# BayesWatch/deep-kernel-transfer

Hardware: AMD Instinct MI355X
Metric: episodes/sec (higher is better)
Workload: dtype f32/f16x2-split

## Files before the change

### deep-kernel-transfer_amd/_lib.py

```python
from __future__ import annotations

import ctypes
import json
import os
import subprocess
import threading
from typing import NamedTuple, Optional

_HERE = os.path.dirname(os.path.abspath(__file__))
_ROOT = os.path.dirname(_HERE)
CSRC = os.path.join(_HERE, "csrc")
INCLUDE = os.path.join(_ROOT, "include")
SOURCES = ["dkt_gram.hip", "dkt_gram_ep.hip", "dkt_gram_big.hip", "dkt_gram_small.hip", "dkt_classkernel.hip", "dkt_mll.hip", "dkt_mll_mfma.hip", "dkt_mll_h2.hip", "dkt_mll_reg.hip", "dkt_mll_big.hip", "dkt_mll_tiled.hip", "dkt_mll_band.hip", "dkt_objective.hip", "dkt_predict.hip",
           "dkt_spectral.hip", "dkt_frontend.hip", "dkt_frontend_big.hip", "dkt_lowrank.hip", "dkt_mll_rownoise.hip", "dkt_laplace_grad.hip"]
OBJ_DIR = os.path.join(_HERE, "build")

_c_p = ctypes.c_void_p
_c_i = ctypes.c_int
_c_f = ctypes.c_float

SIGNATURES = {
    "dkt_abi_version": (_c_i, []),
    "dkt_device_cu_count": (_c_i, []),
    "dkt_reload_env": (None, []),
    "dkt_env_value": (ctypes.c_char_p, [ctypes.c_char_p]),
    "dkt_gram_f32": (_c_i, [_c_p, _c_p, _c_p, _c_i, _c_i, _c_i, _c_i, _c_i, _c_p, _c_p]),
    "dkt_mll_workspace_bytes": (ctypes.c_size_t, [_c_i, _c_i, _c_i]),
    "dkt_mll_workspace_bytes_for": (ctypes.c_size_t, [_c_i, _c_i, _c_i, ctypes.c_uint]),
    "dkt_mll_f32": (_c_i, [_c_p, _c_p, ctypes.c_long, _c_p, _c_p, _c_p, _c_i, _c_i, _c_i, _c_f, _c_i,
                           ctypes.c_uint, _c_p, _c_p, _c_p, _c_p, _c_p, _c_p, _c_p, _c_p, _c_p, _c_p,
                           _c_p, ctypes.c_size_t, _c_p]),
    "dkt_objective_f32": (_c_i, [_c_p, _c_p, _c_p, _c_i, _c_i, _c_p]),
    "dkt_hyper_grads_f32": (_c_i, [_c_p] * 8 + [_c_i, _c_i, _c_p]),
    "dkt_bn_param_grads_workspace_bytes": (ctypes.c_size_t, [_c_i, _c_i]),
    "dkt_bn_param_grads_f32": (_c_i, [_c_p, _c_p, _c_p, _c_p, _c_i, _c_i, _c_p, ctypes.c_size_t, _c_p]),
    "dkt_gram_bwd_f32": (_c_i, [_c_p, _c_p, _c_p, _c_i, _c_i, _c_i, _c_p, ctypes.c_uint, _c_p]),
    "dkt_rbf_bwd_f32": (_c_i, [_c_p, _c_p, _c_p, _c_p, _c_p, _c_i, _c_i, _c_p]),
    "dkt_sqdist_bwd_f32": (_c_i, [_c_p, _c_p, _c_p, _c_p, _c_p, _c_i, _c_i, _c_p]),
    "dkt_predict_f32": (_c_i, [_c_p, _c_p, _c_p, _c_p, _c_p, _c_p, _c_i, _c_i, _c_i, _c_i, _c_p]),
    "dkt_predict_per_class_f32": (_c_i, [_c_p, _c_p, _c_p, _c_p, _c_p, _c_p, _c_i, _c_i, _c_i, _c_i, _c_p]),
    "dkt_predict_var_f32": (_c_i, [_c_p, _c_p, _c_p, _c_p, _c_p, _c_p, _c_i, _c_i, _c_i, _c_i, _c_p]),
    "dkt_bn_stats_f32": (_c_i, [_c_p, _c_p, _c_p, _c_f, _c_p, _c_p, _c_p, _c_p, _c_p, _c_i, _c_i, _c_i, _c_p]),
    "dkt_gram_bn_f32": (_c_i, [_c_p, _c_p, _c_p, ctypes.c_long, _c_p, _c_p, _c_i, _c_i, _c_i, _c_p]),
    "dkt_gram_bn_train_f32": (_c_i, [_c_p, _c_p, _c_p, _c_f, _c_p, _c_p, _c_p, _c_p, _c_p, _c_p, _c_p, _c_i, _c_i, _c_i, _c_p]),
    "dkt_gram_bn_bwd_f32": (_c_i, [_c_p, _c_p, _c_p, _c_p, _c_p, ctypes.c_long, _c_p, _c_p, _c_p, _c_p, _c_p, _c_p, _c_p,
                                   _c_i, _c_i, _c_i, _c_p]),
    "dkt_affine_normalize_f32": (_c_i, [_c_p, _c_p, _c_p, ctypes.c_long, _c_p, _c_p, _c_i, _c_i, _c_i, _c_p]),
    "dkt_normalize_bn_bwd_f32": (_c_i, [_c_p, _c_p, _c_p, _c_p, ctypes.c_long, _c_p, _c_p, _c_p, _c_p, _c_p, _c_p, _c_p, _c_i, _c_i, _c_i, _c_p]),
    "dkt_class_kernel_f32": (_c_i, [_c_p, _c_i, _c_p, _c_i, _c_p, _c_i, _c_i, _c_i, _c_p]),
    "dkt_class_kernel_bwd_nsplit": (_c_i, [_c_i, _c_i]),
    "dkt_class_kernel_bwd_f32": (_c_i, [_c_p, _c_p, _c_i, _c_p, _c_i, _c_p, _c_p, _c_i, _c_i, _c_i, _c_p]),
# ... 550 lines not shown
```

### deep-kernel-transfer_amd/csrc/dkt_common.h

```cpp
#pragma once
#include <hip/hip_runtime.h>
#include <stdint.h>

typedef float f32x4 __attribute__((ext_vector_type(4)));
typedef float f32x16 __attribute__((ext_vector_type(16)));

#define DKT_WAVE 64

#include "dkt_env.h"
#include "dkt_lds_dense.h"

__device__ __forceinline__ float wave_sum(float v) {
#pragma unroll
    for (int o = 32; o > 0; o >>= 1) v += __shfl_down(v, o, DKT_WAVE);
    return v;
}

__device__ __forceinline__ float wave_allsum(float v) {
#pragma unroll
    for (int o = 32; o > 0; o >>= 1) v += __shfl_xor(v, o, DKT_WAVE);
    return v;
}

__device__ __forceinline__ float block_sum_256(float v, float* red) {
    v = wave_sum(v);
    __syncthreads();
    if ((threadIdx.x & 63) == 0) red[threadIdx.x >> 6] = v;
    __syncthreads();
    return red[0] + red[1] + red[2] + red[3];
}

__device__ __forceinline__ float4 load4_guard(const float* row, int col, int ncols, bool row_ok, bool vec_ok) {
    float4 v = make_float4(0.f, 0.f, 0.f, 0.f);
    if (!row_ok) return v;
    if (vec_ok) {
        if (col < ncols) v = *reinterpret_cast<const float4*>(row + col);
    } else {
        if (col + 0 < ncols) v.x = row[col + 0];
        if (col + 1 < ncols) v.y = row[col + 1];
        if (col + 2 < ncols) v.z = row[col + 2];
        if (col + 3 < ncols) v.w = row[col + 3];
    }
    return v;
}

static inline unsigned dkt_lds_pad(DktSwitch pad) { return (unsigned)dkt_env_int(pad, 0); }
```

### deep-kernel-transfer_amd/csrc/dkt_mll.h

```cpp
#pragma once
#include "dkt_common.h"
#include "../../include/dkt_abi.h"

struct MllArgs {
    const float* E;
    const float* Y;
    long y_bstride;
    const float* sv;
    const float* mean;
    const float* noise;
    const float* cls_weight;
    float* logp;
    float* alpha;
    float* L;
    float* W;
    float* dsv;
    float* dmean;
    float* dnoise;
    float* jitter_used;
    int32_t* info;
    float* ws;
    const int32_t* only_failed;
    int b0;
    int B, C, N, LD;
    float jitter0;
    int max_tries;
    unsigned flags;
    int p2_guard;
    float kappa_max = 0.f;
};

constexpr float DKT_HALF_LOG_2PI = 0.91893853320467274178f;
static_assert(DKT_HALF_LOG_2PI == dkt_lds::kHalfLog2Pi, "the two spellings of 1/2 log 2 pi round to one float");

bool dkt_mll_h2_serves(int N, unsigned flags);
void dkt_mll_h2_launch(const MllArgs& a, hipStream_t st);
bool dkt_mll_mfma_serves(int N, unsigned flags);
void dkt_mll_mfma_launch(const MllArgs& a, hipStream_t st);
bool dkt_mll_reg_launch(const MllArgs& a, hipStream_t st);

void dkt_chol_inv_block_launch(const float* A, int lda, long sA, float* L, int ldl, long sL, float* U, int ldu, long sU, int nb,
                               int pivot_base, int32_t* info, int nmat, hipStream_t st);
size_t dkt_mll_big_workspace_bytes(int B, int C, int N);
int dkt_mll_big_launch(const MllArgs& a, void* workspace, size_t ws_bytes, hipStream_t st);
bool dkt_mll_tiled_supports(int N, unsigned flags, int C = 1);
size_t dkt_mll_tiled_workspace_bytes(int B, int C, int N);
size_t dkt_mll_tiled_workspace_bytes_form(int B, int C, int N, bool per_class);
int dkt_mll_tiled_launch(const MllArgs& a, void* workspace, size_t ws_bytes, hipStream_t st);
bool dkt_mll_band_supports(int N, unsigned flags, int C);
bool dkt_mll_band_applies(int B, int C, int N, unsigned flags);
size_t dkt_mll_band_workspace_bytes(int B, int C, int N);
int dkt_mll_band_launch(const MllArgs& a, void* workspace, size_t ws_bytes, hipStream_t st);
void dkt_mll_generic_global_launch(MllArgs a, int b0, int count, float* ws, hipStream_t st);
size_t dkt_mll_generic_global_floats(int count, int N);
```

### deep-kernel-transfer_amd/csrc/dkt_mll.hip

```cpp
#include "dkt_mll.h"
#include <cstdint>
#include <cstdlib>

namespace {

constexpr size_t MLL_LDS_LIMIT = 150 * 1024;

__host__ __device__ inline int mll_ld(int N) { return N | 1; }
inline size_t mll_vec_floats(int N) { return (size_t)3 * (N + 1) + 32; }
inline size_t mll_mat_floats(int N) { return (size_t)(N + 1) * mll_ld(N); }
inline bool mll_fits_lds(int N) { return (mll_vec_floats(N) + mll_mat_floats(N)) * 4 <= MLL_LDS_LIMIT; }

template <bool GLOBAL>
__global__ __launch_bounds__(256) void mll_generic_kernel(MllArgs a) {
    extern __shared__ __attribute__((aligned(16))) float smem[];
    const int tid = threadIdx.x;
    const int tx = tid & 15, ty = tid >> 4;
    const int N = a.N, C = a.C, LD = a.LD, R = N + 1;
    const bool epc = (a.flags & DKT_MLL_E_PER_CLASS) != 0;
    const size_t unit = epc ? (size_t)a.b0 * C + blockIdx.x : (size_t)a.b0 + blockIdx.x;
    const int b = epc ? (int)(unit / (size_t)C) : (int)unit;
    const int c_first = epc ? (int)(unit % (size_t)C) : 0, c_end = epc ? c_first + 1 : C;
    if (a.only_failed) {
        bool need = false;
        for (int c = c_first; c < c_end; ++c) need = need || a.only_failed[(size_t)b * C + c] != 0;
        if (!need) return;
        __syncthreads();
    }
    float* cs = smem;
    float* ldiag = cs + R;
    float* al = ldiag + R;
    float* red = al + R;
    float* Mw = GLOBAL ? (a.ws + (size_t)blockIdx.x * R * LD) : (red + 32);
#define MW(p, j) Mw[(p) * LD + (j)]

    const float* Eb = a.E + unit * N * N;
    const bool want_grad = (a.flags & DKT_MLL_WANT_GRAD) != 0;
    const bool want_chol = (a.flags & DKT_MLL_WANT_CHOL) != 0;
    float* Wb = want_grad ? a.W + unit * N * N : nullptr;

    for (int c = c_first; c < c_end; ++c) {
        const float svc = a.sv[c], mc = a.mean[c], nzc = a.noise[c];
        const float* yc = a.Y + (size_t)b * a.y_bstride + (size_t)c * N;
        int fail_at = 0;
        float jit = 0.f;
        for (int attempt = 0; attempt <= a.max_tries; ++attempt) {
            jit = dkt_jitter_rung(a.jitter0, attempt);
            __syncthreads();
            for (int idx = tid; idx < N * N; idx += 256) {
                const int p = idx / N, j = idx - p * N;
                float v = 0.f;
                if (p >= j) {
// ... 91 lines not shown
                    const float mcv = 0.5f * (al[i] * al[j] - kinv);
                    const float e = Eb[(size_t)i * N + j];
                    if (i == j) { dsv_part += mcv * e; tr_part += mcv; }
                    else dsv_part += 2.0f * mcv * e;
                    const float wv = coef * mcv;
                    if (c == c_first) {
                        Wb[(size_t)i * N + j] = wv;
                        if (i != j) Wb[(size_t)j * N + i] = wv;
                    } else {
                        Wb[(size_t)i * N + j] += wv;
                        if (i != j) Wb[(size_t)j * N + i] += wv;
                    }
                }
            }
            const float dsv = block_sum_256(dsv_part, red);
            const float trm = block_sum_256(tr_part, red);
            if (tid == 0) {
                a.dsv[bc] = dsv;
                a.dmean[bc] = asum;
                a.dnoise[bc] = trm;
            }
        }
    }
#undef MW
}

}

size_t dkt_mll_generic_global_floats(int count, int N) { return (size_t)count * mll_mat_floats(N); }

void dkt_mll_generic_global_launch(MllArgs a, int b0, int count, float* ws, hipStream_t st) {
    a.b0 = b0; a.ws = ws; a.LD = mll_ld(a.N);
    const int units = (a.flags & DKT_MLL_E_PER_CLASS) ? count * a.C : count;
    hipLaunchKernelGGL(mll_generic_kernel<true>, dim3(units), dim3(256), mll_vec_floats(a.N) * sizeof(float), st, a);
}

constexpr float MLL_H2_KAPPA_MAX = 5.0e3f;

static int mll_status() { return hipGetLastError() == hipSuccess ? DKT_OK : DKT_ERR_LAUNCH; }
static int mll_generic_lds_launch(const MllArgs& a, hipStream_t st) {
    const size_t units = (size_t)a.B * ((a.flags & DKT_MLL_E_PER_CLASS) ? a.C : 1);
    const size_t lds = (mll_vec_floats(a.N) + mll_mat_floats(a.N)) * sizeof(float);
    if (lds > 48 * 1024 && hipFuncSetAttribute((const void*)mll_generic_kernel<false>, hipFuncAttributeMaxDynamicSharedMemorySize, (int)lds) != hipSuccess) return DKT_ERR_LAUNCH;
    hipLaunchKernelGGL(mll_generic_kernel<false>, dim3((unsigned)units), dim3(256), lds, st, a);
    return mll_status();
}

static int mll_p2_guard() { return dkt_env_int(DKT_SW_MLL_P2_GUARD, 1); }
static bool mll_force_f32mfma() { return dkt_env_is(DKT_SW_MLL_F32MFMA, '1'); }

enum class MllRoute { BadArg, H2, Mfma, Band, Tiled, Big, GenericLds, GenericGlobal };
struct MllPlan { MllRoute route; size_t ws_bytes; bool kappa_fixup; };

static MllPlan mll_plan(int B, int C, int N, unsigned flags, size_t avail_bytes) {
    if (B <= 0 || C <= 0 || N <= 0) return {MllRoute::BadArg, 0, false};
    const bool pc = (flags & DKT_MLL_E_PER_CLASS) != 0;
    const bool bad = (flags & DKT_MLL_FORCE_REG) || (pc && (flags & (DKT_MLL_WANT_CHOL | DKT_MLL_FORCE_F32MFMA | DKT_MLL_FORCE_BLOCKED)));
    if (mll_force_f32mfma() && !(flags & (DKT_MLL_E_PER_CLASS | DKT_MLL_FORCE_GENERIC | DKT_MLL_FORCE_REG | DKT_MLL_FORCE_BLOCKED))) flags |= DKT_MLL_FORCE_F32MFMA;
    const size_t gen = mll_fits_lds(N) ? 0 : (size_t)(pc ? (B < 128 ? B : 128) * C : B) * mll_mat_floats(N) * sizeof(float);
    MllPlan p = {mll_fits_lds(N) ? MllRoute::GenericLds : MllRoute::GenericGlobal, gen, false};
    size_t ws = 0;
    if (!(flags & DKT_MLL_FORCE_GENERIC)) {
        if (dkt_mll_h2_serves(N, flags)) p = {MllRoute::H2, 0, !(flags & DKT_MLL_NO_KAPPA_GUARD) && mll_fits_lds(N)};
        else if (dkt_mll_mfma_serves(N, flags)) p = {MllRoute::Mfma, 0, false};
        else if (dkt_mll_band_applies(B, C, N, flags) && (ws = dkt_mll_band_workspace_bytes(B, C, N)) <= avail_bytes) p = {MllRoute::Band, ws, false};
        else if (!(flags & DKT_MLL_FORCE_BLOCKED) && dkt_mll_tiled_supports(N, flags, C) && ((ws = dkt_mll_tiled_workspace_bytes_form(B, C, N, pc)) <= avail_bytes || pc))
            p = {MllRoute::Tiled, ws, false};
        else if (!pc && N + 1 > 128 && (ws = dkt_mll_big_workspace_bytes(B, C, N)) <= avail_bytes)
            p = {MllRoute::Big, ws > gen ? ws : gen, false};
    }
    if (bad) p.route = MllRoute::BadArg;
    return p;
}

extern "C" size_t dkt_mll_workspace_bytes(int B, int C, int N) {
    if (B <= 0 || N <= 0 || C <= 0) return 0;
    if (N + 1 <= 128) return 0;
    const size_t big = dkt_mll_big_workspace_bytes(B, C, N);
    const size_t gen = mll_fits_lds(N) ? 0 : (size_t)B * mll_mat_floats(N) * sizeof(float);
    const size_t til = dkt_mll_tiled_supports(N, 0) ? dkt_mll_tiled_workspace_bytes(B, C, N) : 0;
    const size_t bnd = dkt_mll_band_supports(N, 0, C) ? dkt_mll_band_workspace_bytes(B, C, N) : 0;
    size_t mx = big > gen ? big : gen;
    mx = mx > bnd ? mx : bnd;
    return mx > til ? mx : til;
}

extern "C" size_t dkt_mll_workspace_bytes_for(int B, int C, int N, unsigned flags) { return mll_plan(B, C, N, flags, SIZE_MAX).ws_bytes; }

extern "C" int dkt_mll_f32(const float* E, const float* Y, long y_bstride, const float* sv, const float* mean,
                           const float* noise, int B, int C, int N, float jitter0, int max_tries,
                           unsigned flags, const float* cls_weight, float* logp, float* alpha, float* L,
                           float* W, float* dsv, float* dmean, float* dnoise, float* jitter_used,
                           int32_t* info, void* workspace, size_t workspace_bytes, void* stream) {
    if (!E || !Y || !sv || !mean || !noise || !logp || !alpha || !jitter_used || !info) return DKT_ERR_BAD_ARG;
    if (B <= 0 || C <= 0 || N <= 0 || max_tries < 0 || max_tries > 8 || y_bstride < 0) return DKT_ERR_BAD_ARG;
    if ((flags & DKT_MLL_WANT_GRAD) && (!W || !dsv || !dmean || !dnoise)) return DKT_ERR_BAD_ARG;
    if ((flags & DKT_MLL_WANT_CHOL) && !L) return DKT_ERR_BAD_ARG;
    MllArgs a;
    a.E = E; a.Y = Y; a.y_bstride = y_bstride; a.sv = sv; a.mean = mean; a.noise = noise;
    a.cls_weight = cls_weight; a.logp = logp; a.alpha = alpha; a.L = L; a.W = W; a.dsv = dsv;
    a.dmean = dmean; a.dnoise = dnoise; a.jitter_used = jitter_used; a.info = info;
    a.ws = (float*)workspace; a.only_failed = nullptr; a.b0 = 0; a.B = B; a.C = C; a.N = N; a.LD = mll_ld(N);
    a.jitter0 = jitter0; a.max_tries = max_tries; a.flags = flags;
    a.p2_guard = mll_p2_guard();
    hipStream_t st = (hipStream_t)stream;
    const size_t avail = workspace ? workspace_bytes : 0;
    const MllPlan p = mll_plan(B, C, N, flags, avail);
    switch (p.route) {
        case MllRoute::BadArg: return DKT_ERR_BAD_ARG;
        case MllRoute::H2:
            a.kappa_max = p.kappa_fixup ? MLL_H2_KAPPA_MAX : 0.f;
            dkt_mll_h2_launch(a, st);
            if (!p.kappa_fixup) return mll_status();
            a.only_failed = a.info;
            return mll_generic_lds_launch(a, st);
        case MllRoute::Mfma: dkt_mll_mfma_launch(a, st); return mll_status();
        case MllRoute::Band: return dkt_mll_band_launch(a, workspace, workspace_bytes, st);
        case MllRoute::Tiled:
            if (avail < p.ws_bytes) return DKT_ERR_WORKSPACE;
            return dkt_mll_tiled_launch(a, workspace, workspace_bytes, st);
        case MllRoute::Big: return dkt_mll_big_launch(a, workspace, workspace_bytes, st);
        case MllRoute::GenericLds: return mll_generic_lds_launch(a, st);
        case MllRoute::GenericGlobal: {
            const size_t per_ep = (size_t)((flags & DKT_MLL_E_PER_CLASS) ? C : 1) * mll_mat_floats(N) * sizeof(float);
            const size_t fit = avail / per_ep;
            if (fit < 1) return DKT_ERR_WORKSPACE;
            const int cnt = fit < (size_t)B ? (int)fit : B;
            for (int b0 = 0; b0 < B; b0 += cnt) dkt_mll_generic_global_launch(a, b0, (B - b0 < cnt) ? B - b0 : cnt, (float*)workspace, st);
            return mll_status();
        }
    }
    return DKT_ERR_BAD_ARG;
}
```

### deep-kernel-transfer_amd/csrc/dkt_mll_h2.hip

```cpp
#include "dkt_wave_mll.h"
#include <cstdlib>

namespace {

using namespace dkt_mfma;

#ifndef DKT_H2E_P2H
#define DKT_H2E_P2H 1
#endif
#ifndef DKT_H2_SWEEP_PRIO
#define DKT_H2_SWEEP_PRIO 1
#endif

__device__ __forceinline__ void sweep_begin30(const f32x4 S, float (&x)[16], float& dv) {
#pragma unroll
    for (int q = 0; q < 4; ++q) spread_rows(S[q] * TWOM30, x[q], x[4 + q], x[8 + q], x[12 + q]);
    dv = 1.0f;
}

struct P1H2 : P1Base {
    h4 negIh;
};

struct ArithH2 {
// ... 409 lines not shown
            if (round + 1 < nrounds) __syncthreads();
        }
    }
    DKT_CLK(7);
#ifdef DKT_MFMA_CLOCKS
    DKT_CLK(8);
    if ((tid & 63) == 0 && a.ws) {
        unsigned long long* o = reinterpret_cast<unsigned long long*>(a.ws) + ((size_t)blockIdx.x * (MAX_WPG * EPW) + wall) * 48;
        for (int i = 0; i < 32; ++i) o[i] = clk[i];
        for (int i = 0; i < 16; ++i) o[32 + i] = clk2[i];
    }
#endif
}

template <int NT> constexpr int h2e_wlds() { return ntt(NT) < 19 ? ntt(NT) : 19; }

template <int NT>
__global__ __attribute__((amdgpu_flat_work_group_size(64, 64), amdgpu_waves_per_eu(2, 2)))
void mll_h2e_kernel(MllArgs a) {
    constexpr int WLDS = h2e_wlds<NT>();
    constexpr int WREG = ntt(NT) - WLDS;
    __shared__ f32x4 wl[WLDS * 64];
    __shared__ f32x4 yst[NT * 4];

    const bool epc = (a.flags & DKT_MLL_E_PER_CLASS) != 0;
    const bool want_grad = (a.flags & DKT_MLL_WANT_GRAD) != 0;
    const int C = a.C;
    const int b = epc ? (int)(blockIdx.x / (unsigned)C) : (int)blockIdx.x;
    const int c_first = epc ? (int)(blockIdx.x % (unsigned)C) : 0, c_end = epc ? c_first + 1 : C;
    const size_t mat = epc ? (size_t)b * C + c_first : (size_t)b;
    const float qnan = __int_as_float(0x7fc00000);
    int tq = threadIdx.x;
    DKT_OPAQUE_V(tq);
    int c16 = tq & 15, g4 = (tq >> 2) & 12, lane = tq & 63, N = a.N;
    DKT_OPAQUE_S(N);

    f32x4 wr[WREG > 0 ? WREG : 1];
#pragma unroll
    for (int n = 0; n < WREG; ++n) wr[n] = (f32x4){0.f, 0.f, 0.f, 0.f};
#pragma unroll
    for (int n = 0; n < WLDS; ++n) wl[n * 64 + lane] = (f32x4){0.f, 0.f, 0.f, 0.f};
#ifdef DKT_MFMA_CLOCKS
    unsigned long long ph[8] = {}, tprev = __builtin_amdgcn_s_memtime();
#define DKT_PH(i) do { __builtin_amdgcn_sched_barrier(0); const unsigned long long tn = __builtin_amdgcn_s_memtime(); ph[i] += tn - tprev; tprev = tn; __builtin_amdgcn_sched_barrier(0); } while (0)
#else
#define DKT_PH(i) do { } while (0)
// ... 387 lines not shown
        if (want_grad && !live && fail_at == 0) {
            float fro = 0.f;
#pragma unroll
            for (int j = 0; j < NT; ++j) {
#pragma unroll
                for (int i = 0; i <= j; ++i) {
#if DKT_H2E_P2H
                    const f32x4 u = join_h2(T.t[i][j]);
#else
                    const f32x4 u = T.t[i][j];
#endif
#pragma unroll
                    for (int q = 0; q < 4; ++q) fro += (j < NT - 1 || g4 + q < pN) ? u[q] * u[q] : 0.f;
                }
            }
#if DKT_H2E_P2H
            trk = wave_reduce_dpp<false>(fro) * ldexpf(1.0f, -2 * msc) / (gsc * gsc * unit2 * unit2) - aa;
#else
            trk = wave_reduce_dpp<false>(fro) * ldexpf(1.0f, -2 * msc) - aa;
#endif
        }
        if (lane == 0) {
            const bool ok = fail_at == 0;
            a.logp[bc] = ok ? (-0.5f * quad - 0.34657359027997264f * lsum - (float)N * DKT_HALF_LOG_2PI) : qnan;
            a.jitter_used[bc] = jit;
            a.info[bc] = (ok && kappa_high) ? -1 : fail_at;
            if (want_grad) {
                const float nz_eff = nzc + jit;
                a.dmean[bc] = ok ? asum : qnan;
                a.dnoise[bc] = ok ? -0.5f * trk : qnan;
                a.dsv[bc] = ok ? 0.5f * ((quad - (float)N) + nz_eff * trk) / svc : qnan;
            }
        }
        DKT_PH(5);
        attempt = 0;
        ++c;
    }
    if (want_grad) {
        tq = threadIdx.x;
        DKT_OPAQUE_V(tq);
        c16 = tq & 15; g4 = (tq >> 2) & 12; lane = tq & 63; N = a.N;
        DKT_OPAQUE_S(N);
        const int pN = N - 16 * (NT - 1);
        const float fin = poison ? qnan : ((sigma == 0.f) ? 0.f : sigma * ldexpf(1.0f, -2 * (15 - e_acc)));
        const brsrc Wr = mk_rsrc(a.W + mat * N * N, (unsigned)(N * N * 4));
#pragma unroll
        for (int j = 0; j < NT; ++j) {
            const bool col_ok = (j < NT - 1) || (c16 < pN);
#pragma unroll
            for (int i = 0; i <= j; ++i) {
                const int n = tidx(i, j);
                f32x4 v;
                if (n < WLDS) v = wl[n * 64 + lane];
                else v = wr[n - WLDS < 0 ? 0 : n - WLDS];
#pragma unroll
                for (int q = 0; q < 4; ++q) v[q] = poison ? qnan : v[q] * fin;
                if (i < j) {
                    bstore4(Wr, v, col_ok ? ((16 * j + c16) * N + 16 * i + g4) * 4 : OOB, 0);
#pragma unroll
                    for (int q = 0; q < 4; ++q) {
// ... 12 lines not shown
            }
        }
    }
#ifdef DKT_MFMA_CLOCKS
    DKT_PH(6);
    if (lane == 0 && a.ws) {
        unsigned long long* o = reinterpret_cast<unsigned long long*>(a.ws) + (size_t)blockIdx.x * 8;
        for (int i = 0; i < 7; ++i) o[i] = ph[i];
        o[7] = __builtin_amdgcn_s_getreg((4 << 0) | (0 << 6) | (31 << 11));
    }
#endif
}

int h2e_min_batch() { return dkt_env_int(DKT_SW_MLL_H2E_MINB, 1024); }

template <int NT>
void launch_h2(const MllArgs& a, hipStream_t st) {
    const bool g = (a.flags & DKT_MLL_WANT_GRAD) != 0;
    if constexpr (NT <= 7) {
        if (a.flags & DKT_MLL_E_PER_CLASS) {
            hipLaunchKernelGGL((mll_h2e_kernel<NT>), dim3(a.B * a.C), dim3(64), 0, st, a);
            return;
        }
        if (g && a.B >= h2e_min_batch()) {
            hipLaunchKernelGGL((mll_h2e_kernel<NT>), dim3(a.B), dim3(64), 0, st, a);
            return;
        }
    }
    const bool epc = (a.flags & DKT_MLL_E_PER_CLASS) != 0;
    const int rounds = (a.C + MAX_WPG - 1) / MAX_WPG;
    const int wpg = epc ? 1 : (a.C + rounds - 1) / rounds;
    constexpr int EPW = epw<NT>();
    const dim3 grid(((epc ? a.B * a.C : a.B) + EPW - 1) / EPW), block(64 * wpg * EPW);
    if (g && wpg == 5) hipLaunchKernelGGL((mll_h2_kernel<NT, true, true>), grid, block, 0, st, a, wpg);
    else if (g) hipLaunchKernelGGL((mll_h2_kernel<NT, true, false>), grid, block, 0, st, a, wpg);
    else hipLaunchKernelGGL((mll_h2_kernel<NT, false, false>), grid, block, 0, st, a, wpg);
}

}

bool dkt_mll_h2_serves(int N, unsigned flags) { return N + 1 <= 128 && !(flags & (DKT_MLL_WANT_CHOL | DKT_MLL_FORCE_F32MFMA)); }

void dkt_mll_h2_launch(const MllArgs& a, hipStream_t st) {
    switch ((a.N + 1 + 15) / 16) {
        case 1: launch_h2<1>(a, st); break;
        case 2: launch_h2<2>(a, st); break;
        case 3: launch_h2<3>(a, st); break;
        case 4: launch_h2<4>(a, st); break;
        case 5: launch_h2<5>(a, st); break;
        case 6: launch_h2<6>(a, st); break;
        case 7: launch_h2<7>(a, st); break;
        case 8: launch_h2<8>(a, st); break;
        default: break;
    }
}
```

### deep-kernel-transfer_amd/csrc/dkt_objective.hip

```cpp
#include "dkt_common.h"
#include "../../include/dkt_abi.h"

namespace {

__global__ __launch_bounds__(256) void objective_kernel(const float* __restrict__ logp, const float* __restrict__ cw, float* __restrict__ obj, const int B, const int C) {
    const int b = blockIdx.x * 256 + threadIdx.x;
    if (b >= B) return;
    float s = 0.f;
    for (int c = 0; c < C; ++c) s += (cw ? cw[c] : 1.0f) * logp[(size_t)b * C + c];
    obj[b] = s;
}

__global__ __launch_bounds__(256) void hyper_grads_kernel(const float* __restrict__ gobj, const float* __restrict__ cw, const float* __restrict__ d0, const float* __restrict__ d1,
                                                          const float* __restrict__ d2, float* __restrict__ g0, float* __restrict__ g1, float* __restrict__ g2, const int B,
                                                          const int C) {
    __shared__ float red[256];
    const int c = blockIdx.x, which = blockIdx.y, tid = threadIdx.x;
    const float* d = which == 0 ? d0 : (which == 1 ? d1 : d2);
    float* g = which == 0 ? g0 : (which == 1 ? g1 : g2);
    if (!d || !g) return;
    float s = 0.f;
    for (int b = tid; b < B; b += 256) s += gobj[b] * d[(size_t)b * C + c];
    red[tid] = s;
    __syncthreads();
#pragma unroll
    for (int w = 128; w > 0; w >>= 1) {
        if (tid < w) red[tid] += red[tid + w];
        __syncthreads();
    }
    if (tid == 0) g[c] = (cw ? cw[c] : 1.0f) * red[0];
}

// ... 85 lines not shown
```

### deep-kernel-transfer_amd/ops.py

```python
from __future__ import annotations

import ctypes
import os
import re
from typing import Optional

import torch

from . import _lib

KERNEL_LINEAR = 0
KERNEL_RBF = 1
KERNEL_SQDIST = 2
KERNEL_LINEAR_UNIT = 3
GRAM_UNIT_ROWS = 1
GRAM_W_SYMMETRIC = 2
MLL_WANT_GRAD = 1
MLL_WANT_CHOL = 2
MLL_FORCE_GENERIC = 4
MLL_FORCE_REG = 8
MLL_FORCE_BLOCKED = 16
MLL_FORCE_F32MFMA = 32
MLL_E_PER_CLASS = 64
MLL_FORCE_TILED = 128
MLL_FORCE_BAND = 256
MLL_NO_KAPPA_GUARD = 512

LINEAR_KINDS = ("linear", "cossim", "bncossim")
RBF_KINDS = ("rbf", "RBF")
MATERN_KINDS = ("matern",)
POLY_KINDS = {"poli1": 1, "poli2": 2}


def kind_id(kernel: str) -> int:
    if kernel in LINEAR_KINDS:
        return KERNEL_LINEAR
    if kernel in RBF_KINDS:
        return KERNEL_RBF
    raise ValueError("[ERROR] the kernel '" + str(kernel) + "' is not supported!")


def _req(t: torch.Tensor, name: str, ndim: Optional[int] = None) -> torch.Tensor:
    if not isinstance(t, torch.Tensor) or not t.is_cuda:
        raise RuntimeError("dkt_amd.ops: `%s` must be a CUDA/ROCm tensor -- the DKT hot path is HIP-only "
                           "(no CPU fallback)" % name)
    if t.dtype != torch.float32:
        raise RuntimeError("dkt_amd.ops: `%s` must be float32, got %s" % (name, t.dtype))
    if ndim is not None and t.dim() != ndim:
        raise RuntimeError("dkt_amd.ops: `%s` must have %d dims, got %s" % (name, ndim, tuple(t.shape)))
# ... 104 lines not shown
         lengthscale: Optional[torch.Tensor] = None) -> torch.Tensor:
    a = _req(a, "a", 3)
    b_, m, d = a.shape
    if bm is not None:
        bm = _req(bm, "bm", 3)
        if bm.shape[0] != b_ or bm.shape[2] != d:
            raise RuntimeError("gram: shape mismatch %s vs %s" % (tuple(a.shape), tuple(bm.shape)))
        n = bm.shape[1]
    else:
        n = m
    if kind not in (KERNEL_LINEAR, KERNEL_LINEAR_UNIT):
        lengthscale = _req(lengthscale.reshape(-1), "lengthscale", 1)
    e = torch.empty((b_, m, n), device=a.device, dtype=torch.float32)
    lib = _lib_now()
    with _timed("dkt_gram_f32"):
        st = lib.dkt_gram_f32(_p(a), _p(bm), _p(e), b_, m, n, d, kind, _p(lengthscale), _stream())
    _lib.check(st, "dkt_gram_f32")
    return e


def mll(e: torch.Tensor, y: torch.Tensor, sv: torch.Tensor, mean: torch.Tensor, noise: torch.Tensor,
        want_grad: bool = False, want_chol: bool = False, cls_weight: Optional[torch.Tensor] = None,
        jitter0: float = 1e-6, max_tries: int = 3, force_generic: bool = False, force_reg: bool = False,
        force_blocked: bool = False, force_f32mfma: bool = False, force_tiled: bool = False, force_band: bool = False, no_kappa_guard: bool = False) -> dict:
    per_class = e.dim() == 4
    e = _req(e, "e", 4 if per_class else 3)
    b_, n, n2 = e.shape[0], e.shape[-2], e.shape[-1]
    if n != n2:
        raise RuntimeError("mll: e must be [B,N,N] or [B,C,N,N]")
    y = _req(y, "y")
    if y.dim() == 2:
        c_, y_bstride = y.shape[0], 0
    elif y.dim() == 3 and y.shape[0] == b_:
        c_, y_bstride = y.shape[1], y.shape[1] * n
    else:
        raise RuntimeError("mll: y must be [C,N] or [B,C,N]")
    if y.shape[-1] != n:
        raise RuntimeError("mll: y last dim %d != N %d" % (y.shape[-1], n))
    sv = _req(sv.reshape(-1), "sv", 1)
    mean = _req(mean.reshape(-1), "mean", 1)
    noise = _req(noise.reshape(-1), "noise", 1)
    if not (sv.numel() == mean.numel() == noise.numel() == c_):
        raise RuntimeError("mll: sv/mean/noise must have C=%d elements" % c_)
    if per_class and e.shape[1] != c_:
        raise RuntimeError("mll: per-class e must be [B,C=%d,N,N]" % c_)
    dev = e.device
    logp = torch.empty((b_, c_), device=dev, dtype=torch.float32)
# ... 2 lines not shown
    info = torch.empty((b_, c_), device=dev, dtype=torch.int32)
    flags = ((MLL_FORCE_GENERIC if force_generic else 0) | (MLL_FORCE_BLOCKED if force_blocked else 0) |
             (MLL_FORCE_F32MFMA if force_f32mfma else 0) | (MLL_E_PER_CLASS if per_class else 0) | (MLL_FORCE_TILED if force_tiled else 0) | (MLL_FORCE_BAND if force_band else 0) | (MLL_NO_KAPPA_GUARD if no_kappa_guard else 0))
    chol = w = dsv = dmean = dnoise = None
    if want_chol:
        flags |= MLL_WANT_CHOL
        chol = torch.empty((b_, c_, n, n), device=dev, dtype=torch.float32)
    if want_grad:
        flags |= MLL_WANT_GRAD
        w = torch.empty((b_, c_, n, n) if per_class else (b_, n, n), device=dev, dtype=torch.float32)
        dsv = torch.empty((b_, c_), device=dev, dtype=torch.float32)
        dmean = torch.empty((b_, c_), device=dev, dtype=torch.float32)
        dnoise = torch.empty((b_, c_), device=dev, dtype=torch.float32)
    if cls_weight is not None:
        cls_weight = _req(cls_weight.reshape(-1), "cls_weight", 1)
    if force_reg and n + 1 <= 128:
        if per_class or force_generic or force_blocked or force_f32mfma:
            raise RuntimeError("mll: force_reg combines with want_grad / want_chol only")
        dlib = _lib.load_diag()
        st = dlib.dkt_diag_mll_reg_f32(_p(e), _p(y), y_bstride, _p(sv), _p(mean), _p(noise), b_, c_, n, float(jitter0), int(max_tries),
                                       flags & (MLL_WANT_GRAD | MLL_WANT_CHOL), _p(cls_weight), _p(logp), _p(alpha), _p(chol), _p(w), _p(dsv), _p(dmean), _p(dnoise),
                                       _p(jit), _p(info), _stream())
        _lib.check(st, "dkt_diag_mll_reg_f32")
        return dict(logp=logp, alpha=alpha, jitter=jit, info=info, chol=chol, w=w, dsv=dsv, dmean=dmean, dnoise=dnoise)
    lib = _lib_now(want_twin=force_f32mfma)
    ws_bytes = int(lib.dkt_mll_workspace_bytes_for(b_, c_, n, flags))
    ws = torch.empty((max(ws_bytes, 4) + 3) // 4, device=dev, dtype=torch.float32) if ws_bytes else None
    with _timed("dkt_mll_f32"):
        st = lib.dkt_mll_f32(_p(e), _p(y), y_bstride, _p(sv), _p(mean), _p(noise), b_, c_, n,
                             float(jitter0), int(max_tries), flags, _p(cls_weight), _p(logp), _p(alpha),
                             _p(chol), _p(w), _p(dsv), _p(dmean), _p(dnoise), _p(jit), _p(info), _p(ws),
                             ws_bytes, _stream())
    _lib.check(st, "dkt_mll_f32")
    return dict(logp=logp, alpha=alpha, jitter=jit, info=info, chol=chol, w=w, dsv=dsv, dmean=dmean, dnoise=dnoise)


def gram_bwd(w: torch.Tensor, z: torch.Tensor, ep_scale: Optional[torch.Tensor] = None, unit_rows: bool = False,
             w_symmetric: bool = False) -> torch.Tensor:
    w = _req(w, "w", 3)
    z = _req(z, "z", 3)
    b_, n, d = z.shape
    if tuple(w.shape) != (b_, n, n):
        raise RuntimeError("gram_bwd: w must be [B,N,N]")
    if ep_scale is not None:
        ep_scale = _req(ep_scale.reshape(-1), "ep_scale", 1)
        if ep_scale.numel() != b_:
            raise RuntimeError("gram_bwd: ep_scale must have B elements")
    dz = torch.empty_like(z)
    lib = _lib_now()
    with _timed("dkt_gram_bwd_f32"):
        st = lib.dkt_gram_bwd_f32(_p(w), _p(z), _p(dz), b_, n, d, _p(ep_scale),
                                  (GRAM_UNIT_ROWS if unit_rows else 0) | (GRAM_W_SYMMETRIC if w_symmetric else 0), _stream())
    _lib.check(st, "dkt_gram_bwd_f32")
    return dz


def _req_distance_bwd(fn: str, w: torch.Tensor, m: torch.Tensor, mname: str, lengthscale: torch.Tensor):
# ... 911 lines not shown
    stride = _ab_stride(a, a, b_, d)
    train = mean is not None
    if train:
        mean = _req(mean, "mean", 2)
        rstd = _req(rstd, "rstd", 2)
    dx = torch.empty_like(x)
    dg = torch.empty((b_, d), device=x.device, dtype=torch.float32) if train else None
    db = torch.empty((b_, d), device=x.device, dtype=torch.float32) if train else None
    ws = torch.empty((b_, n), device=x.device, dtype=torch.float32)
    _front_end("normalize_bn_bwd", x, [_p(dzn), _p(zn), _p(x), _p(a), stride, _p(mean), _p(rstd), _p(rnorm), _p(dx), _p(dg), _p(db), _p(ws), b_, n, d,
                                       _stream()], 2)
    return dx, dg, db


def _sum_episodes(gobj: torch.Tensor, part: torch.Tensor, shape) -> torch.Tensor:
    return (gobj.reshape(-1, 1) * part).sum(0).reshape(shape)


class _Gaussian:
    on_features = resident_only = False

    @staticmethod
    def forward(e, y, sv, mean, noise, cls_weight, jitter0, max_tries):
        out = mll(e, y, sv, mean, noise, want_grad=True, cls_weight=cls_weight, jitter0=jitter0, max_tries=max_tries)
        obj = objective(out["logp"], cls_weight)
        return (obj, (out["logp"], out["alpha"], out["info"], out["jitter"]), (out["w"], out["dsv"], out["dmean"], out["dnoise"], cls_weight),
                (sv.shape, mean.shape, noise.shape))

    @staticmethod
    def de(saved):
        w, *_ = saved
        return w

    @staticmethod
    def backward(saved, shapes, gobj, need_y, need_sv, need_mean, need_noise, *_):
        *_, dsv, dmean, dnoise, cw = saved
        return (None,) + hyper_grads(gobj, cw, dsv if need_sv else None, dmean if need_mean else None, dnoise if need_noise else None, shapes) + (None, None, None)


class _LooCV(_Gaussian):
    on_features, resident_only = False, True

    @staticmethod
    def forward(e, y, sv, mean, noise, cls_weight, jitter0, max_tries):
        with torch.no_grad():
            out = loo(e, y, sv, mean, noise, want_grad=True, cls_weight=cls_weight, jitter0=jitter0, max_tries=max_tries)
            obj = objective(out["loo"], cls_weight)
        return (obj, (out["loo"], out["alpha"], out["info"], out["jitter"], out["mu_loo"], out["var_loo"]),
# ... 290 lines not shown
```

### include/dkt_abi.h

```cpp
#ifndef DKT_ABI_H
#define DKT_ABI_H

#include <stddef.h>
#include <stdint.h>

#ifdef __cplusplus
extern "C" {
#endif

#define DKT_ABI_VERSION 8

#define DKT_OK 0
#define DKT_ERR_BAD_ARG (-1)
#define DKT_ERR_TOO_LARGE (-2)
#define DKT_ERR_WORKSPACE (-3)
#define DKT_ERR_LAUNCH (-4)
#ifndef DKT_ERR_SHAPE
#define DKT_ERR_SHAPE (-5)
#endif

#define DKT_KERNEL_LINEAR 0
#define DKT_KERNEL_RBF 1
#define DKT_KERNEL_SQDIST 2
#define DKT_KERNEL_LINEAR_UNIT 3

#define DKT_GRAM_UNIT_ROWS 1u
#define DKT_GRAM_W_SYMMETRIC 2u

#define DKT_MLL_WANT_GRAD 1u
#define DKT_MLL_WANT_CHOL 2u
#define DKT_MLL_FORCE_GENERIC 4u
#define DKT_MLL_FORCE_REG 8u
#define DKT_MLL_FORCE_BLOCKED 16u
#define DKT_MLL_FORCE_F32MFMA 32u
#define DKT_MLL_FORCE_TILED 128u
#define DKT_MLL_FORCE_BAND 256u
#define DKT_MLL_NO_KAPPA_GUARD 512u
#define DKT_MLL_E_PER_CLASS 64u

int dkt_abi_version(void);


void dkt_reload_env(void);
const char* dkt_env_value(const char* name);

int dkt_device_cu_count(void);

int dkt_gram_f32(const float* A, const float* Bm, float* E, int B, int M, int N, int D, int kind,
                 const float* lengthscale, void* stream);

size_t dkt_mll_workspace_bytes(int B, int C, int N);
size_t dkt_mll_workspace_bytes_for(int B, int C, int N, unsigned flags);

int dkt_mll_f32(const float* E, const float* Y, long y_bstride, const float* sv, const float* mean,
                const float* noise, int B, int C, int N, float jitter0, int max_tries,
                unsigned flags, const float* cls_weight, float* logp, float* alpha, float* L,
                float* W, float* dsv, float* dmean, float* dnoise, float* jitter_used,
                int32_t* info, void* workspace, size_t workspace_bytes, void* stream);

int dkt_gram_bwd_f32(const float* W, const float* Z, float* dZ, int B, int N, int D,
                     const float* ep_scale, unsigned flags, void* stream);

int dkt_rbf_bwd_f32(const float* W, const float* E, const float* lengthscale, float* Wp,
                    float* dlengthscale, int B, int N, void* stream);

int dkt_objective_f32(const float* logp, const float* cls_weight, float* obj, int B, int C, void* stream);
int dkt_hyper_grads_f32(const float* gobj, const float* cls_weight, const float* dsv, const float* dmean, const float* dnoise,
                        float* gsv, float* gmean, float* gnoise, int B, int C, void* stream);

int dkt_sqdist_bwd_f32(const float* W, const float* U, const float* lengthscale, float* Wp,
                       float* dlengthscale, int B, int N, void* stream);

int dkt_predict_f32(const float* Ex, const float* alpha, const float* sv, const float* mean,
                    float* mu, int32_t* labels, int B, int C, int M, int N, void* stream);

// ... 86 lines not shown
```

Before: 2.048 million.

## Fuse weighted objective reduction into H2 MLL kernel and batch fixup walk

Computes the per-episode class-weighted objective inside the wave-per-episode H2 MLL kernel, reusing the otherwise-null L pointer as the output, so the separate objective kernel launch is skipped. The kappa fixup pass through the generic kernel now walks 16 episodes per block using a failure bitmask and also rewrites the objective for the episodes it recomputes. This is meant to cut launch overhead and the extra pass over logp. In exchange it adds ABI surface, a new flag and an env switch, and the fixup grid now serialises up to 16 episodes per block.

```diff
diff --git a/deep-kernel-transfer_amd/_lib.py b/deep-kernel-transfer_amd/_lib.py
--- a/deep-kernel-transfer_amd/_lib.py
+++ b/deep-kernel-transfer_amd/_lib.py
@@ -27,6 +27,7 @@
     "dkt_gram_f32": (_c_i, [_c_p, _c_p, _c_p, _c_i, _c_i, _c_i, _c_i, _c_i, _c_p, _c_p]),
     "dkt_mll_workspace_bytes": (ctypes.c_size_t, [_c_i, _c_i, _c_i]),
     "dkt_mll_workspace_bytes_for": (ctypes.c_size_t, [_c_i, _c_i, _c_i, ctypes.c_uint]),
+    "dkt_mll_obj_supported": (_c_i, [_c_i, _c_i, _c_i, ctypes.c_uint]),
     "dkt_mll_f32": (_c_i, [_c_p, _c_p, ctypes.c_long, _c_p, _c_p, _c_p, _c_i, _c_i, _c_i, _c_f, _c_i,
                            ctypes.c_uint, _c_p, _c_p, _c_p, _c_p, _c_p, _c_p, _c_p, _c_p, _c_p, _c_p,
                            _c_p, ctypes.c_size_t, _c_p]),
diff --git a/deep-kernel-transfer_amd/csrc/dkt_common.h b/deep-kernel-transfer_amd/csrc/dkt_common.h
--- a/deep-kernel-transfer_amd/csrc/dkt_common.h
+++ b/deep-kernel-transfer_amd/csrc/dkt_common.h
@@ -30,6 +30,8 @@
     return red[0] + red[1] + red[2] + red[3];
 }
 
+__device__ __forceinline__ float dkt_objective_add(float s, float cw, float logp) { return __builtin_fmaf(cw, logp, s); }
+
 __device__ __forceinline__ float4 load4_guard(const float* row, int col, int ncols, bool row_ok, bool vec_ok) {
     float4 v = make_float4(0.f, 0.f, 0.f, 0.f);
     if (!row_ok) return v;
diff --git a/deep-kernel-transfer_amd/csrc/dkt_mll.h b/deep-kernel-transfer_amd/csrc/dkt_mll.h
--- a/deep-kernel-transfer_amd/csrc/dkt_mll.h
+++ b/deep-kernel-transfer_amd/csrc/dkt_mll.h
@@ -28,12 +28,16 @@
     unsigned flags;
     int p2_guard;
     float kappa_max = 0.f;
+    float* obj = nullptr;
+    int walk = 0;
+    int nunits = 0;
 };
 
 constexpr float DKT_HALF_LOG_2PI = 0.91893853320467274178f;
 static_assert(DKT_HALF_LOG_2PI == dkt_lds::kHalfLog2Pi, "the two spellings of 1/2 log 2 pi round to one float");
 
 bool dkt_mll_h2_serves(int N, unsigned flags);
+bool dkt_mll_h2_wave_per_episode(int B, int N, unsigned flags);
 void dkt_mll_h2_launch(const MllArgs& a, hipStream_t st);
 bool dkt_mll_mfma_serves(int N, unsigned flags);
 void dkt_mll_mfma_launch(const MllArgs& a, hipStream_t st);
diff --git a/deep-kernel-transfer_amd/csrc/dkt_mll.hip b/deep-kernel-transfer_amd/csrc/dkt_mll.hip
--- a/deep-kernel-transfer_amd/csrc/dkt_mll.hip
+++ b/deep-kernel-transfer_amd/csrc/dkt_mll.hip
@@ -18,16 +18,35 @@
     const int tx = tid & 15, ty = tid >> 4;
     const int N = a.N, C = a.C, LD = a.LD, R = N + 1;
     const bool epc = (a.flags & DKT_MLL_E_PER_CLASS) != 0;
-    const size_t unit = epc ? (size_t)a.b0 * C + blockIdx.x : (size_t)a.b0 + blockIdx.x;
+    float* cs = smem;
+    const unsigned x0 = a.walk > 0 ? blockIdx.x * (unsigned)a.walk : blockIdx.x;
+    unsigned todo = 1u;
+    if (a.walk > 0) {
+        const int per = epc ? 1 : C;
+        const int nfl = min(a.walk, a.nunits - (int)x0) * per;
+        const int32_t* fl = a.only_failed + (epc ? (size_t)a.b0 * C + x0 : ((size_t)a.b0 + x0) * C);
+        unsigned m = 0u;
+        for (int i = tid; i < nfl; i += 256) m |= (fl[i] != 0) ? 1u << (i / per) : 0u;
+#pragma unroll
+        for (int o = 32; o > 0; o >>= 1) m |= (unsigned)__shfl_xor((int)m, o, DKT_WAVE);
+        unsigned* wm = reinterpret_cast<unsigned*>(cs);
+        if ((tid & 63) == 0) wm[tid >> 6] = m;
+        __syncthreads();
+        todo = wm[0] | wm[1] | wm[2] | wm[3];
+        __syncthreads();
+    }
+    for (unsigned xi = 0; todo != 0u; ++xi, todo >>= 1) {
+    if (!(todo & 1u)) continue;
+    const unsigned x = x0 + xi;
+    const size_t unit = epc ? (size_t)a.b0 * C + x : (size_t)a.b0 + x;
     const int b = epc ? (int)(unit / (size_t)C) : (int)unit;
     const int c_first = epc ? (int)(unit % (size_t)C) : 0, c_end = epc ? c_first + 1 : C;
-    if (a.only_failed) {
+    if (a.only_failed && a.walk <= 0) {
         bool need = false;
         for (int c = c_first; c < c_end; ++c) need = need || a.only_failed[(size_t)b * C + c] != 0;
         if (!need) return;
         __syncthreads();
     }
-    float* cs = smem;
     float* ldiag = cs + R;
     float* al = ldiag + R;
     float* red = al + R;
@@ -165,6 +184,12 @@
             }
         }
     }
+    if (a.obj && tid == 0) {
+        float s = 0.f;
+        for (int c = 0; c < C; ++c) s = dkt_objective_add(s, a.cls_weight ? a.cls_weight[c] : 1.0f, a.logp[(size_t)b * C + c]);
+        a.obj[b] = s;
+    }
+    }
 #undef MW
 }
 
@@ -179,13 +204,15 @@
 }
 
 constexpr float MLL_H2_KAPPA_MAX = 5.0e3f;
+constexpr int MLL_FIXUP_WALK = 16;
 
 static int mll_status() { return hipGetLastError() == hipSuccess ? DKT_OK : DKT_ERR_LAUNCH; }
 static int mll_generic_lds_launch(const MllArgs& a, hipStream_t st) {
     const size_t units = (size_t)a.B * ((a.flags & DKT_MLL_E_PER_CLASS) ? a.C : 1);
     const size_t lds = (mll_vec_floats(a.N) + mll_mat_floats(a.N)) * sizeof(float);
     if (lds > 48 * 1024 && hipFuncSetAttribute((const void*)mll_generic_kernel<false>, hipFuncAttributeMaxDynamicSharedMemorySize, (int)lds) != hipSuccess) return DKT_ERR_LAUNCH;
-    hipLaunchKernelGGL(mll_generic_kernel<false>, dim3((unsigned)units), dim3(256), lds, st, a);
+    const unsigned grid = a.walk > 0 ? (unsigned)((units + a.walk - 1) / a.walk) : (unsigned)units;
+    hipLaunchKernelGGL(mll_generic_kernel<false>, dim3(grid), dim3(256), lds, st, a);
     return mll_status();
 }
 
@@ -193,7 +220,7 @@
 static bool mll_force_f32mfma() { return dkt_env_is(DKT_SW_MLL_F32MFMA, '1'); }
 
 enum class MllRoute { BadArg, H2, Mfma, Band, Tiled, Big, GenericLds, GenericGlobal };
-struct MllPlan { MllRoute route; size_t ws_bytes; bool kappa_fixup; };
+struct MllPlan { MllRoute route; size_t ws_bytes; bool kappa_fixup; bool wave_per_episode = false; };
 
 static MllPlan mll_plan(int B, int C, int N, unsigned flags, size_t avail_bytes) {
     if (B <= 0 || C <= 0 || N <= 0) return {MllRoute::BadArg, 0, false};
@@ -204,7 +231,7 @@
     MllPlan p = {mll_fits_lds(N) ? MllRoute::GenericLds : MllRoute::GenericGlobal, gen, false};
     size_t ws = 0;
     if (!(flags & DKT_MLL_FORCE_GENERIC)) {
-        if (dkt_mll_h2_serves(N, flags)) p = {MllRoute::H2, 0, !(flags & DKT_MLL_NO_KAPPA_GUARD) && mll_fits_lds(N)};
+        if (dkt_mll_h2_serves(N, flags)) p = {MllRoute::H2, 0, !(flags & DKT_MLL_NO_KAPPA_GUARD) && mll_fits_lds(N), dkt_mll_h2_wave_per_episode(B, N, flags)};
         else if (dkt_mll_mfma_serves(N, flags)) p = {MllRoute::Mfma, 0, false};
         else if (dkt_mll_band_applies(B, C, N, flags) && (ws = dkt_mll_band_workspace_bytes(B, C, N)) <= avail_bytes) p = {MllRoute::Band, ws, false};
         else if (!(flags & DKT_MLL_FORCE_BLOCKED) && dkt_mll_tiled_supports(N, flags, C) && ((ws = dkt_mll_tiled_workspace_bytes_form(B, C, N, pc)) <= avail_bytes || pc))
@@ -230,6 +257,11 @@
 
 extern "C" size_t dkt_mll_workspace_bytes_for(int B, int C, int N, unsigned flags) { return mll_plan(B, C, N, flags, SIZE_MAX).ws_bytes; }
 
+extern "C" int dkt_mll_obj_supported(int B, int C, int N, unsigned flags) {
+    const MllPlan p = mll_plan(B, C, N, flags & ~DKT_MLL_FUSED_EPILOGUE, SIZE_MAX);
+    return p.route == MllRoute::H2 && p.wave_per_episode;
+}
+
 extern "C" int dkt_mll_f32(const float* E, const float* Y, long y_bstride, const float* sv, const float* mean,
                            const float* noise, int B, int C, int N, float jitter0, int max_tries,
                            unsigned flags, const float* cls_weight, float* logp, float* alpha, float* L,
@@ -239,6 +271,9 @@
     if (B <= 0 || C <= 0 || N <= 0 || max_tries < 0 || max_tries > 8 || y_bstride < 0) return DKT_ERR_BAD_ARG;
     if ((flags & DKT_MLL_WANT_GRAD) && (!W || !dsv || !dmean || !dnoise)) return DKT_ERR_BAD_ARG;
     if ((flags & DKT_MLL_WANT_CHOL) && !L) return DKT_ERR_BAD_ARG;
+    const bool fused = (flags & DKT_MLL_FUSED_EPILOGUE) != 0;
+    if (fused && !L) return DKT_ERR_BAD_ARG;
+    flags &= ~DKT_MLL_FUSED_EPILOGUE;
     MllArgs a;
     a.E = E; a.Y = Y; a.y_bstride = y_bstride; a.sv = sv; a.mean = mean; a.noise = noise;
     a.cls_weight = cls_weight; a.logp = logp; a.alpha = alpha; a.L = L; a.W = W; a.dsv = dsv;
@@ -249,13 +284,16 @@
     hipStream_t st = (hipStream_t)stream;
     const size_t avail = workspace ? workspace_bytes : 0;
     const MllPlan p = mll_plan(B, C, N, flags, avail);
+    if (fused && !(p.route == MllRoute::H2 && p.wave_per_episode)) return DKT_ERR_BAD_ARG;
     switch (p.route) {
         case MllRoute::BadArg: return DKT_ERR_BAD_ARG;
         case MllRoute::H2:
             a.kappa_max = p.kappa_fixup ? MLL_H2_KAPPA_MAX : 0.f;
+            if (fused) { a.L = nullptr; a.obj = L; }
             dkt_mll_h2_launch(a, st);
             if (!p.kappa_fixup) return mll_status();
             a.only_failed = a.info;
+            if (fused) { a.walk = MLL_FIXUP_WALK; a.nunits = B; }
             return mll_generic_lds_launch(a, st);
         case MllRoute::Mfma: dkt_mll_mfma_launch(a, st); return mll_status();
         case MllRoute::Band: return dkt_mll_band_launch(a, workspace, workspace_bytes, st);
diff --git a/deep-kernel-transfer_amd/csrc/dkt_mll_h2.hip b/deep-kernel-transfer_amd/csrc/dkt_mll_h2.hip
--- a/deep-kernel-transfer_amd/csrc/dkt_mll_h2.hip
+++ b/deep-kernel-transfer_amd/csrc/dkt_mll_h2.hip
@@ -455,6 +455,7 @@
     constexpr int WREG = ntt(NT) - WLDS;
     __shared__ f32x4 wl[WLDS * 64];
     __shared__ f32x4 yst[NT * 4];
+    __shared__ float objs;
 
     const bool epc = (a.flags & DKT_MLL_E_PER_CLASS) != 0;
     const bool want_grad = (a.flags & DKT_MLL_WANT_GRAD) != 0;
@@ -888,7 +889,9 @@
         }
         if (lane == 0) {
             const bool ok = fail_at == 0;
-            a.logp[bc] = ok ? (-0.5f * quad - 0.34657359027997264f * lsum - (float)N * DKT_HALF_LOG_2PI) : qnan;
+            const float lp = ok ? (-0.5f * quad - 0.34657359027997264f * lsum - (float)N * DKT_HALF_LOG_2PI) : qnan;
+            a.logp[bc] = lp;
+            if (a.obj) objs = dkt_objective_add(c == c_first ? 0.f : objs, a.cls_weight ? a.cls_weight[c] : 1.0f, lp);
             a.jitter_used[bc] = jit;
             a.info[bc] = (ok && kappa_high) ? -1 : fail_at;
             if (want_grad) {
@@ -902,6 +905,7 @@
         attempt = 0;
         ++c;
     }
+    if (a.obj && threadIdx.x == 0) a.obj[b] = objs;
     if (want_grad) {
         tq = threadIdx.x;
         DKT_OPAQUE_V(tq);
@@ -960,7 +964,7 @@
             hipLaunchKernelGGL((mll_h2e_kernel<NT>), dim3(a.B * a.C), dim3(64), 0, st, a);
             return;
         }
-        if (g && a.B >= h2e_min_batch()) {
+        if (dkt_mll_h2_wave_per_episode(a.B, a.N, a.flags)) {
             hipLaunchKernelGGL((mll_h2e_kernel<NT>), dim3(a.B), dim3(64), 0, st, a);
             return;
         }
@@ -978,6 +982,10 @@
 }
 
 bool dkt_mll_h2_serves(int N, unsigned flags) { return N + 1 <= 128 && !(flags & (DKT_MLL_WANT_CHOL | DKT_MLL_FORCE_F32MFMA)); }
+
+bool dkt_mll_h2_wave_per_episode(int B, int N, unsigned flags) {
+    return dkt_mll_h2_serves(N, flags) && N + 1 <= 16 * 7 && (flags & DKT_MLL_WANT_GRAD) && !(flags & DKT_MLL_E_PER_CLASS) && B >= h2e_min_batch();
+}
 
 void dkt_mll_h2_launch(const MllArgs& a, hipStream_t st) {
     switch ((a.N + 1 + 15) / 16) {
diff --git a/deep-kernel-transfer_amd/csrc/dkt_objective.hip b/deep-kernel-transfer_amd/csrc/dkt_objective.hip
--- a/deep-kernel-transfer_amd/csrc/dkt_objective.hip
+++ b/deep-kernel-transfer_amd/csrc/dkt_objective.hip
@@ -7,7 +7,7 @@
     const int b = blockIdx.x * 256 + threadIdx.x;
     if (b >= B) return;
     float s = 0.f;
-    for (int c = 0; c < C; ++c) s += (cw ? cw[c] : 1.0f) * logp[(size_t)b * C + c];
+    for (int c = 0; c < C; ++c) s = dkt_objective_add(s, cw ? cw[c] : 1.0f, logp[(size_t)b * C + c]);
     obj[b] = s;
 }
 
diff --git a/deep-kernel-transfer_amd/ops.py b/deep-kernel-transfer_amd/ops.py
--- a/deep-kernel-transfer_amd/ops.py
+++ b/deep-kernel-transfer_amd/ops.py
@@ -25,6 +25,7 @@
 MLL_FORCE_TILED = 128
 MLL_FORCE_BAND = 256
 MLL_NO_KAPPA_GUARD = 512
+MLL_FUSED_EPILOGUE = 1024
 
 LINEAR_KINDS = ("linear", "cossim", "bncossim")
 RBF_KINDS = ("rbf", "RBF")
@@ -175,7 +176,8 @@
 def mll(e: torch.Tensor, y: torch.Tensor, sv: torch.Tensor, mean: torch.Tensor, noise: torch.Tensor,
         want_grad: bool = False, want_chol: bool = False, cls_weight: Optional[torch.Tensor] = None,
         jitter0: float = 1e-6, max_tries: int = 3, force_generic: bool = False, force_reg: bool = False,
-        force_blocked: bool = False, force_f32mfma: bool = False, force_tiled: bool = False, force_band: bool = False, no_kappa_guard: bool = False) -> dict:
+        force_blocked: bool = False, force_f32mfma: bool = False, force_tiled: bool = False, force_band: bool = False, no_kappa_guard: bool = False,
+        want_obj: bool = False) -> dict:
     per_class = e.dim() == 4
     e = _req(e, "e", 4 if per_class else 3)
     b_, n, n2 = e.shape[0], e.shape[-2], e.shape[-1]
@@ -224,9 +226,13 @@
                                        flags & (MLL_WANT_GRAD | MLL_WANT_CHOL), _p(cls_weight), _p(logp), _p(alpha), _p(chol), _p(w), _p(dsv), _p(dmean), _p(dnoise),
                                        _p(jit), _p(info), _stream())
         _lib.check(st, "dkt_diag_mll_reg_f32")
-        return dict(logp=logp, alpha=alpha, jitter=jit, info=info, chol=chol, w=w, dsv=dsv, dmean=dmean, dnoise=dnoise)
+        return dict(logp=logp, alpha=alpha, jitter=jit, info=info, chol=chol, w=w, dsv=dsv, dmean=dmean, dnoise=dnoise, obj=None)
     lib = _lib_now(want_twin=force_f32mfma)
-    ws_bytes = int(lib.dkt_mll_workspace_bytes_for(b_, c_, n, flags))
+    obj = None
+    if want_obj and not force_reg and lib.dkt_mll_obj_supported(b_, c_, n, flags):
+        flags |= MLL_FUSED_EPILOGUE
+        chol = obj = torch.empty((b_,), device=dev, dtype=torch.float32)
+    ws_bytes = int(lib.dkt_mll_workspace_bytes_for(b_, c_, n, flags & ~MLL_FUSED_EPILOGUE))
     ws = torch.empty((max(ws_bytes, 4) + 3) // 4, device=dev, dtype=torch.float32) if ws_bytes else None
     with _timed("dkt_mll_f32"):
         st = lib.dkt_mll_f32(_p(e), _p(y), y_bstride, _p(sv), _p(mean), _p(noise), b_, c_, n,
@@ -234,7 +240,7 @@
                              _p(chol), _p(w), _p(dsv), _p(dmean), _p(dnoise), _p(jit), _p(info), _p(ws),
                              ws_bytes, _stream())
     _lib.check(st, "dkt_mll_f32")
-    return dict(logp=logp, alpha=alpha, jitter=jit, info=info, chol=chol, w=w, dsv=dsv, dmean=dmean, dnoise=dnoise)
+    return dict(logp=logp, alpha=alpha, jitter=jit, info=info, chol=None if obj is not None else chol, w=w, dsv=dsv, dmean=dmean, dnoise=dnoise, obj=obj)
 
 
 def gram_bwd(w: torch.Tensor, z: torch.Tensor, ep_scale: Optional[torch.Tensor] = None, unit_rows: bool = False,
@@ -1192,8 +1198,9 @@
 
     @staticmethod
     def forward(e, y, sv, mean, noise, cls_weight, jitter0, max_tries):
-        out = mll(e, y, sv, mean, noise, want_grad=True, cls_weight=cls_weight, jitter0=jitter0, max_tries=max_tries)
-        obj = objective(out["logp"], cls_weight)
+        fused = os.environ.get("DKT_FUSED_EPILOGUE", "1") != "0" and os.environ.get("DKT_FUSED_REDUCTIONS", "1") != "0"
+        out = mll(e, y, sv, mean, noise, want_grad=True, cls_weight=cls_weight, jitter0=jitter0, max_tries=max_tries, want_obj=fused)
+        obj = out["obj"] if out["obj"] is not None else objective(out["logp"], cls_weight)
         return (obj, (out["logp"], out["alpha"], out["info"], out["jitter"]), (out["w"], out["dsv"], out["dmean"], out["dnoise"], cls_weight),
                 (sv.shape, mean.shape, noise.shape))
 
diff --git a/include/dkt_abi.h b/include/dkt_abi.h
--- a/include/dkt_abi.h
+++ b/include/dkt_abi.h
@@ -37,6 +37,7 @@
 #define DKT_MLL_FORCE_BAND 256u
 #define DKT_MLL_NO_KAPPA_GUARD 512u
 #define DKT_MLL_E_PER_CLASS 64u
+#define DKT_MLL_FUSED_EPILOGUE 1024u
 
 int dkt_abi_version(void);
 
@@ -51,6 +52,7 @@
 
 size_t dkt_mll_workspace_bytes(int B, int C, int N);
 size_t dkt_mll_workspace_bytes_for(int B, int C, int N, unsigned flags);
+int dkt_mll_obj_supported(int B, int C, int N, unsigned flags);
 
 int dkt_mll_f32(const float* E, const float* Y, long y_bstride, const float* sv, const float* mean,
                 const float* noise, int B, int C, int N, float jitter0, int max_tries,
```

New measurement: 2.052 million (median of 6 runs). No clear change (+0.2%).
